# ERGO-Code/ipx

Hardware: AMD Instinct MI355X
Metric: kkt_solves_per_sec (higher is better)
Workload: dtype f64; 1 GPU; C3 synthetic LP m=1000000 n=2000000 8 nnz/col (nnz=16000000), KKTSolverDiag::Solve = diag-precond CR to tol=0.3*sqrt(mu), scaling spread s=1; rows of AI partitioned over 1 GPU(s); errflag=0

## Files before the change

ipx_amd/csrc/api.hip:

```cpp

#include <algorithm>
#include <map>
#include <thread>

#include "context.hpp"

namespace ipxk {

static thread_local std::string g_last_error;
void set_last_error(const std::string& msg) { g_last_error = msg; }

Context::~Context() {
    if (split) destroy_split(split);
    if (split_spare) destroy_split(split_spare);
    if (prepare_host) destroy_prepare_host(prepare_host);
    if (lu) destroy_lu(lu);
    if (maxvol) destroy_maxvol(maxvol);
    if (nmat) destroy_nmatrix(nmat);
    comm_destroy(this);
    if (h_state) (void)hipHostFree(h_state);
    if (h_cycle_done) (void)hipHostFree(h_cycle_done);
    if (ev_a) (void)hipEventDestroy(ev_a);
    if (ev_b) (void)hipEventDestroy(ev_b);
    for (hipEvent_t e : ev_window) (void)hipEventDestroy(e);
// ... 1200 lines not shown
        for (int i = 0; i < 48; i++) info[i] = 0;
        const SpmvLayout L = M.layout;
        info[0] = M.tile_base() != SpmvLayout::phased; info[2] = L == SpmvLayout::sortedfused; info[3] = M.nlong;
        info[4] = M.sliced.built; info[5] = M.sliced.R; info[6] = M.sliced.nslices; info[7] = M.sliced.nrb;
        info[8] = M.sliced.nrows_pad; info[9] = M.sliced.max_tile;
        { double d = M.sliced.dominant_fraction; memcpy(&info[10], &d, sizeof d); }
        info[11] = M.sorted.built; info[14] = M.sorted.nrb;
        info[15] = M.sorted.RB; info[16] = M.sorted.nrows_pad; info[17] = M.sorted.max_sub;
        info[20] = M.nnz;
        info[21] = M.P; info[22] = M.G; info[23] = (ipxint)M.RT * 1000000 + (ipxint)M.Q * 1000 + 0;
        info[24] = L == SpmvLayout::acc; info[25] = M.acc.built; info[26] = M.acc.nslices; info[27] = M.acc.nrb; info[28] = M.acc.RB;
        info[29] = M.acc.nrows_pad; info[30] = M.acc.slice_elems; info[31] = M.acc.nbatches; info[32] = M.acc.deferred;
        info[33] = L == SpmvLayout::accfused; info[34] = M.accf.built; info[35] = M.accf.nrb; info[36] = M.accf.RB; info[37] = M.accf.nbatches;
        info[38] = L == SpmvLayout::plain; info[39] = M.acc.nsteps;
        info[40] = M.acc.wide_units;
        if (create_ms) for (int i = 0; i < 4; i++) create_ms[i] = c->create_ms[i];
    });
}
int ipxk_layout_array(ipxk_context* c, int which, int array, void* out, ipxint cap, ipxint* nbytes) {
    return guarded([&] {
        IPXK_REQUIRE(c && nbytes && (which == 0 || which == 1), "bad argument");
        bind_device(c);
        const GatherMatrix& M = which == 0 ? c->Acols : c->Arows;
        const void* src = nullptr;
        size_t bytes = 0;
        const size_t ntiles = (size_t)M.sliced.nrb * M.sliced.nslices, nsorted = (size_t)M.sorted.nrb;
        const size_t nz = (size_t)M.nnz;
        switch (array) {
            case 0: src = M.sliced.tile_ptr.get(); bytes = M.sliced.built ? (ntiles + 1) * 4 : 0; break;
            case 1: src = M.sliced.cnt.get(); bytes = M.sliced.built ? ntiles * M.sliced.R : 0; break;
// ... 88 lines not shown
```

ipx_amd/csrc/context.hpp:

```cpp
#pragma once

#include "internal.hpp"
#include "device_utils.hpp"

struct ncclComm;

namespace ipxk {

constexpr int kPartialStride = kMaxPartials + 8;

enum PartialSlot {
    kPartRes0 = 0,
    kPartRes1,
    kPartPdot,
    kPartCdot,
    kPartRsdot,
    kPartScratch,
    kNumPartialSlots
};

struct Reordered {
    bool active = false;
    int levels = 0;
    int components = 0;
// ... 57 lines not shown
    DevBuf<int> schur_colptr;
    DevBuf<int> chol_info;
    DevBuf<unsigned char> dense_mask;
    std::vector<int> dense_rank_k;
    DevBuf<double> dense_W, dense_Wsend, dense_Wrecv;
    DevBuf<int> dense_Widx;

    DevBuf<double> v_rhs, v_lhs, v_residual, v_sresidual, v_step, v_Cstep, v_Cres, v_pCstep;
    DevBuf<double> v_resscale_in;
    DevBuf<double> partials;
    DevBuf<CrState> state;
    CrState* h_state = nullptr;
    DevBuf<double> hist;
    hipEvent_t ev_a = nullptr, ev_b = nullptr;
    std::vector<hipEvent_t> ev_window;

    DevBuf<double> resscale;
    DevBuf<double> k_a, k_b, k_x, k_y;
    DevBuf<double> k_tmp;
    bool kkt_diag_factorized = false;

    DevBuf<double> nw_rhs1, nw_rhs2;
    DevBuf<double> nw_in[10], nw_out[6];
    DevBuf<unsigned char> nw_state;

    DevBuf<double> it_x, it_xl, it_xu, it_y, it_zl, it_zu, it_partials;
    DevBuf<double> it_row, it_bnd, it_table;
    DevBuf<unsigned char> it_state;
    bool it_set = false;
    DevBuf<double> ipm[12];
// ... 67 lines not shown
void reorder_permute_weights(Context* c, const double* W_old, double* W_new);

void dense_lu_inverse(Context* c, int kb, const double* D, const double* invL, const double* invU, double* X, double* Xt, int refine = 0);

enum TimeKind { kTimeOp = 0, kTimePrecond = 1, kTimeB = 2, kTimeBt = 3, kNumTimeKinds = 4 };
void time_mark(Context* c, int kind, bool begin);
void time_start(Context* c, ipxk_times* times);
void time_collect(Context* c, ipxk_times* times);

const double* stage_in(Context* c, const double* p, size_t len, DevBuf<double>& buf);
double* stage_out(Context* c, double* p, size_t len, DevBuf<double>& buf);
void finish_out(Context* c, double* user, const double* dev, size_t len);

void normal_apply_dev(Context* c, const double* W, const double* rhs, double* lhs, int* ndot,
                      const int* done);
float time_normal_pair(Context* c, GatherMatrix& Ac, GatherMatrix& Ar);
void debug_single_pass(Context* c, int which, const double* x, double* out);

void prepare_dense_columns(Context* c);
void reset_dense_columns(Context* c);
void diag_factorize_dev(Context* c, const double* W, bool precond_dense_cols, ipxint* errflag);
int diag_apply_dev(Context* c, const double* rhs, double* lhs, int slot, const int* done);

struct CrResult { ipxint iter; ipxint errflag; };
CrResult pcr_solve_dev(Context* c, const double* rhs, double tol, const double* resscale,
                       ipxint maxiter, double* lhs, bool lhs_is_zero, ipxk_interrupt_fn interrupt,
                       void* user, double* hist_host, ipxint hist_cap, ipxk_times* times);
CrResult cr_solve_dev(Context* c, const double* rhs, double tol, const double* resscale,
                      ipxint maxiter, double* lhs, bool lhs_is_zero, ipxk_interrupt_fn interrupt,
                      void* user, double* hist_host, ipxint hist_cap, ipxk_times* times);
// ... 180 lines not shown
```

ipx_amd/csrc/cr.hip:

```cpp
#include <cmath>

#include "context.hpp"
#include "spmv_kernels.hpp"

namespace ipxk {

constexpr int kWindow = 2;

enum CrMode { kModePcrDiag = 0, kModePcrSmw = 1, kModePlain = 2 };

constexpr int kCrUnroll = 4;

struct CrVecs {
    int m;
    double* lhs;
    double* residual;
    double* sresidual;
    double* step;
    double* Cstep;
    double* Cres;
    double* pCstep;
    const double* resscale;
    const double* diag;
};
// ... 23 lines not shown
        st->maxiter = maxiter;
        st->k_started = 0;
        st->k_finished = 0;
        st->cdot[0] = st->cdot[1] = 0.0;
        st->rps[0] = r;
        st->rps[1] = 0.0;
        st->resnorm = 0.0;
        st->iter = 0;
        st->errflag = 0;
        st->done = 0;
        st->hist_cap = hist_cap;
        st->diag_rps_old = st->diag_rps_new = 0.0;
        st->mode = mode;
        st->alpha_pending = 0.0;
        st->k_pending = -1;
    }
}

struct CtlGroup {
    double q[kCrUnroll], r[kCrUnroll], sr[kCrUnroll], d[kCrUnroll], sc[kCrUnroll], s[kCrUnroll], l[kCrUnroll];
};
template <int MODE>
__device__ __forceinline__ void ctl_load(const CrVecs& v, int lazy, long long i0, long long stride, long long last, CtlGroup& g) {
#pragma unroll
    for (int u = 0; u < kCrUnroll; u++) {
        const long long i = min(i0 + u * stride, last);
        g.q[u] = v.Cstep[i];
        g.r[u] = v.residual[i];
        if (MODE != kModePlain) g.sr[u] = v.sresidual[i];
        if (MODE == kModePcrDiag) g.d[u] = v.diag[i];
// ... 208 lines not shown
    for (; i0 < v.m; i0 += kCrUnroll * stride) {
        DirGroup g{};
        dir_load<MODE, INIT>(v, src, owed, i0, stride, last, g);
        dir_update<MODE, INIT>(v, owed, alpha, beta, i0, stride, last, g, acc);
    }
    if (MODE != kModePcrSmw) {
        acc = block_reduce<SumOp>(acc, red);
        if (threadIdx.x == 0) pdot_partial[blockIdx.x] = acc;
    }
    if (blockIdx.x == 0 && threadIdx.x == 0) {
        st->cdot[(k + 1) & 1] = cdotnew;
        st->k_finished = k + 1;
    }
}

__global__ __launch_bounds__(kBlock) void cr_flush_update_kernel(const CrState* st, CrVecs v) {
    if (st->k_pending < 0 || st->k_pending != st->k_finished) return;
    const double alpha = st->alpha_pending;
    for (int i = blockIdx.x * kBlock + threadIdx.x; i < v.m; i += gridDim.x * kBlock) v.lhs[i] += alpha * v.step[i];
}

__global__ __launch_bounds__(kBlock) void finalize_scalar_kernel(PartRef ref, int op, double* out) {
    __shared__ double red[kBlock / 64 + 1];
    const double v = op == 1 ? reduce_partials<MaxOp>(ref, red)
                   : op == 2 ? reduce_partials<MinOp>(ref, red) : reduce_partials<SumOp>(ref, red);
    if (threadIdx.x == 0) *out = v;
}

__global__ void snapshot_done_kernel(const CrState* st, int* host_slot) {
    __hip_atomic_store(host_slot, st->done, __ATOMIC_RELAXED, __HIP_MEMORY_SCOPE_SYSTEM);
// ... 10 lines not shown
constexpr int kDoneRing = kWindow + 2;
constexpr int kDoneNow = 2 * kDoneRing;

static bool cr_lazy() {
    static const bool setting = [] { const char* e = getenv("IPXK_CR_LAZY"); return !e || atoi(e) != 0; }();
    return setting;
}

static bool cr_early() {
    static const bool setting = [] { const char* e = getenv("IPXK_CR_EARLY"); return !e || atoi(e) != 0; }();
    return setting;
}

static int cr_grid_cap() {
    static const int setting = [] { const char* e = getenv("IPXK_CR_GRID"); return e ? atoi(e) : 0; }();
    return setting;
}

static void ensure_comm_buffers(Context* c) {
    if (c->comm_scalars.size() < 64) c->comm_scalars.resize(64);
    if (c->comm_send.size() < (size_t)kNumPartialSlots) {
        c->comm_send.resize(kNumPartialSlots);
        IPXK_HIP(hipMemsetAsync(c->comm_send.get(), 0, sizeof(double) * kNumPartialSlots, c->stream));
    }
    const size_t need = (size_t)c->nranks * kNumPartialSlots;
    if (c->comm_gather.size() < need) c->comm_gather.resize(need);
}

struct Pub {
    Context* c;
// ... 69 lines not shown

struct CrOps {
    int mode;
    int (*applyC)(Context*, const double* rhs, double* lhs, const int* done);
};

static int applyC_normal(Context* c, const double* rhs, double* lhs, const int* done) {
    int np = 0;
    time_mark(c, kTimeOp, true);
    normal_apply_dev(c, c->W, rhs, lhs, &np, done);
    time_mark(c, kTimeOp, false);
    return np;
}
static int applyC_split(Context* c, const double* rhs, double* lhs, const int* done) {
    return split_apply_dev(c, rhs, lhs, done);
}

template <int MODE>
static CrResult run_cr(Context* c, const CrOps& ops, const double* rhs, double tol,
                       const double* resscale, ipxint maxiter, double* lhs, bool lhs_is_zero,
                       ipxk_interrupt_fn interrupt, void* user, double* hist_host, ipxint hist_cap,
                       ipxk_times* times) {
    ensure_workspaces(c);
    time_start(c, times);
    hipStream_t s = c->stream;
    const int m = (int)c->m;
    if (maxiter < 0) maxiter = (comm_active(c) ? c->m_global : c->m) + 100;
    if (hist_cap < 0) hist_cap = 0;
    if (!hist_host) hist_cap = 0;
    if (c->hist.size() < (size_t)hist_cap + 1) c->hist.resize((size_t)hist_cap + 1);
    CrState* st = c->state.get();
    int* done = &st->done;
    const int g = cr_grid_cap() > 0 ? std::min(vec_grid(m), cr_grid_cap()) : vec_grid(m);
    const Pub pub(c);
    for (int i = 0; i <= kDoneNow; i++) c->h_cycle_done[i] = 0;
    const bool multi = comm_active(c);
    const int lazy = cr_lazy() ? 1 : 0;
    const bool early = cr_early() && m > 0;
    const auto control = early ? cr_control_update_kernel<MODE, true> : cr_control_update_kernel<MODE, false>;
    const auto direction0 = early ? cr_direction_kernel<MODE, true, true> : cr_direction_kernel<MODE, true, false>;
    const auto direction = early ? cr_direction_kernel<MODE, false, true> : cr_direction_kernel<MODE, false, false>;
    int* done_now = multi ? nullptr : c->d_cycle_done + kDoneNow;
    if (multi) ensure_comm_buffers(c);

    CrVecs v;
    v.m = m; v.lhs = lhs; v.residual = c->v_residual.get(); v.sresidual = c->v_sresidual.get();
    v.step = c->v_step.get(); v.Cstep = c->v_Cstep.get(); v.Cres = c->v_Cres.get();
    v.pCstep = c->v_pCstep.get(); v.resscale = resscale; v.diag = c->reord.in_use ? c->reord.diagonal.get() : c->diagonal.get();

    IPXK_HIP(hipEventRecord(c->ev_a, s));

    if (lhs_is_zero) {
        hipLaunchKernelGGL(residual_init_kernel, dim3(g), dim3(kBlock), 0, s, m, rhs,
                           (const double*)nullptr, resscale, v.residual, c->part(kPartRes0));
    } else {
        ops.applyC(c, lhs, v.Cres, nullptr);
        hipLaunchKernelGGL(residual_init_kernel, dim3(g), dim3(kBlock), 0, s, m, rhs,
                           (const double*)v.Cres, resscale, v.residual, c->part(kPartRes0));
// ... 6 lines not shown
    const PartRef rsdot = MODE != kModePlain ? pub.ref(kPartRsdot, nrsdot) : PartRef{nullptr, 0, 1};
    hipLaunchKernelGGL(cr_init_state_kernel, dim3(1), dim3(kBlock), 0, s, st, tol, (long long)maxiter,
                       (long long)hist_cap, rsdot, (int)MODE);
    const double* csrc = MODE == kModePlain ? v.residual : v.sresidual;
    int ncdot = ops.applyC(c, csrc, v.Cres, nullptr);
    pub.publish(kPartCdot, ncdot, 0);
    hipLaunchKernelGGL(direction0, dim3(g), dim3(kBlock), 0, s, st, v,
                       pub.ref(kPartCdot, ncdot), c->part(kPartPdot));
    int npdot = g;
    if (MODE == kModePcrSmw) npdot = diag_apply_dev(c, v.Cstep, v.pCstep, kPartPdot, nullptr);
    pub.publish(kPartPdot, npdot, 0);
    const PartRef pdot_ref = pub.ref(kPartPdot, npdot);

    ipxint interrupt_flag = 0, my_interrupt = 0;
    bool agreed_done = false, tail = false;
    for (long long cycle = 0;; cycle++) {
        const long long k0 = cycle * 5;
        if (k0 > maxiter) break;
        if (cycle >= kWindow) {
            const long long cw = cycle - kWindow;
            IPXK_HIP(hipEventSynchronize(c->ev_window[cw % (kWindow + 1)]));
            if (*(volatile int*)(c->h_cycle_done + cw % kDoneRing)) { agreed_done = true; break; }
            if (multi) {
                const int agreed = *(volatile int*)(c->h_cycle_done + kDoneRing + cw % kDoneRing);
                if (agreed != 0) { interrupt_flag = agreed; break; }
            }
        }
        if (interrupt && cycle > 0) {
            my_interrupt = interrupt(user);
            if (!multi && my_interrupt != 0) { interrupt_flag = my_interrupt; break; }
        }
        for (long long k = k0; k < k0 + 5 && k <= maxiter; k++) {
            if (done_now && *(volatile int*)(c->h_cycle_done + kDoneNow)) tail = true;
            if (tail) break;
            hipLaunchKernelGGL(control, dim3(g), dim3(kBlock), 0, s, st, v,
                               res0, res1, pdot_ref, rsdot, c->part(kPartRes0), c->part(kPartRes1),
                               c->hist.get(), lazy, done_now);
            ncdot = ops.applyC(c, csrc, v.Cres, done);
            pub.publish(kPartCdot, ncdot, 0, ((k + 1) & 1) ? kPartRes1 : kPartRes0, g, 1);
            hipLaunchKernelGGL(direction, dim3(g), dim3(kBlock), 0, s, st, v,
                               pub.ref(kPartCdot, ncdot), c->part(kPartPdot));
            if (MODE == kModePcrSmw) diag_apply_dev(c, v.Cstep, v.pCstep, kPartPdot, done);
            if (MODE != kModePlain && (k + 1) % 5 == 0) {
                diag_apply_dev(c, v.residual, v.sresidual, kPartRsdot, done);
                pub.publish(kPartPdot, npdot, 0, kPartRsdot, nrsdot, 0);
            } else {
                pub.publish(kPartPdot, npdot, 0);
            }
        }
        if (multi) {
            double* flags = c->comm_scalars.get() + 56;
            hipLaunchKernelGGL(cycle_flags_kernel, dim3(1), dim3(1), 0, s, st, (double)my_interrupt, flags);
            comm_allreduce_max(c, flags, 2);
            hipLaunchKernelGGL(snapshot_flags_kernel, dim3(1), dim3(1), 0, s, flags, c->d_cycle_done + cycle % kDoneRing,
                               c->d_cycle_done + kDoneRing + cycle % kDoneRing);
        } else {
            hipLaunchKernelGGL(snapshot_done_kernel, dim3(1), dim3(1), 0, s, st, c->d_cycle_done + cycle % kDoneRing);
        }
        IPXK_HIP(hipEventRecord(c->ev_window[cycle % (kWindow + 1)], s));
    }
    if (lazy) hipLaunchKernelGGL(cr_flush_update_kernel, dim3(g), dim3(kBlock), 0, s, st, v);
    IPXK_HIP(hipEventRecord(c->ev_b, s));
    IPXK_HIP(hipMemcpyAsync(c->h_state, st, sizeof(CrState), hipMemcpyDeviceToHost, s));
    IPXK_HIP(hipStreamSynchronize(s));
    IPXK_HIP(hipGetLastError());
    comm_check(c);

    if (multi && agreed_done && !c->h_state->done)
        throw Error(IPXK_E_HIP, "ranks of a partitioned solve diverged (another rank finished the CR loop, this one did not)");
    CrResult res;
    if (c->h_state->done) {
        res.iter = c->h_state->iter;
        res.errflag = c->h_state->errflag;
    } else {
        res.iter = c->h_state->k_finished;
        res.errflag = interrupt_flag;
    }
    if (hist_cap > 0) {
        long long nh = c->h_state->done && c->h_state->errflag != 204 ? res.iter + 1 : res.iter;
        if (!c->h_state->done) nh = c->h_state->k_started;
        if (nh > hist_cap) nh = hist_cap;
// ... 71 lines not shown
```

ipx_amd/csrc/device_utils.hpp:

```cpp
#pragma once

#include <hip/hip_runtime.h>

#include <climits>

#include "internal.hpp"

#define IPXK_GRID_STRIDE(i, n) for (int64_t i = (int64_t)blockIdx.x * blockDim.x + threadIdx.x; i < (n); i += (int64_t)gridDim.x * blockDim.x)

namespace ipxk {

template <class T>
__global__ void fill_kernel(int64_t n, T v, T* __restrict__ a) { IPXK_GRID_STRIDE(i, n) a[i] = v; }

template <int kThreads>
__global__ __launch_bounds__(kThreads) void scan_u32_kernel(int n, const unsigned* __restrict__ in, unsigned* __restrict__ out) {
    __shared__ unsigned wsum[kThreads / 64];
    __shared__ unsigned carry;
    const int tid = threadIdx.x, lane = tid & 63, wave = tid >> 6;
    if (tid == 0) carry = 0;
    __syncthreads();
    for (int base = 0; base < n; base += kThreads) {
        const int i = base + tid;
        const unsigned v = i < n ? in[i] : 0u;
// ... 118 lines not shown
__device__ __forceinline__ void block_argmax(double& v, int& i) {
    __shared__ double sv[kThreads / 64];
    __shared__ int si[kThreads / 64];
    wave_argmax(v, i);
    if ((threadIdx.x & 63) == 0) { sv[threadIdx.x >> 6] = v; si[threadIdx.x >> 6] = i; }
    __syncthreads();
    if (threadIdx.x == 0)
        for (int k = 1; k < kThreads / 64; k++) take_larger(v, i, sv[k], si[k]);
}
template <int kBest>
__device__ __forceinline__ Partial<kBest> load_partial(int nparts, const Partial<kBest>* part) {
    return (int)threadIdx.x < nparts ? part[threadIdx.x] : partial_identity<kBest>();
}

template <class Op>
__device__ __forceinline__ double block_reduce(double v, double* scratch) {
    const int lane = threadIdx.x & 63, wave = threadIdx.x >> 6;
    v = wave_reduce<Op>(v);
    __syncthreads();
    if (lane == 0) scratch[wave] = v;
    __syncthreads();
    double r = scratch[0];
#pragma unroll
    for (int w = 1; w < kBlock / 64; w++) r = Op::apply(r, scratch[w]);
    return r;
}

struct PartRef {
    const double* p;
    int count;
    int stride;
};

constexpr int kPartialsPerThread = kMaxPartials / kBlock;

__device__ __forceinline__ void load_partials(PartRef part, double (&v)[kPartialsPerThread]) {
    const int last = max(part.count - 1, 0);
#pragma unroll
    for (int j = 0; j < kPartialsPerThread; j++)
        v[j] = part.p[(size_t)min((int)threadIdx.x + j * kBlock, last) * part.stride];
}
template <class Op>
__device__ __forceinline__ double fold_partials(PartRef part, const double (&v)[kPartialsPerThread]) {
    double r = Op::identity();
#pragma unroll
    for (int j = 0; j < kPartialsPerThread; j++)
        if ((int)threadIdx.x + j * kBlock < part.count) r = Op::apply(r, v[j]);
    for (int i = threadIdx.x + kMaxPartials; i < part.count; i += kBlock)
        r = Op::apply(r, part.p[(size_t)i * part.stride]);
    return r;
}

template <class Op>
__device__ __forceinline__ double reduce_partials(PartRef part, double* scratch) {
    double v[kPartialsPerThread];
    load_partials(part, v);
    return block_reduce<Op>(fold_partials<Op>(part, v), scratch);
}

template <class OpA, class OpB>
__device__ __forceinline__ void block_reduce2(double& va, double& vb, double* scratch_a, double* scratch_b) {
    const int lane = threadIdx.x & 63, wave = threadIdx.x >> 6;
    va = wave_reduce<OpA>(va);
    vb = wave_reduce<OpB>(vb);
    __syncthreads();
    if (lane == 0) { scratch_a[wave] = va; scratch_b[wave] = vb; }
    __syncthreads();
    double ra = scratch_a[0], rb = scratch_b[0];
#pragma unroll
    for (int w = 1; w < kBlock / 64; w++) { ra = OpA::apply(ra, scratch_a[w]); rb = OpB::apply(rb, scratch_b[w]); }
    va = ra;
    vb = rb;
}
template <class OpA, class OpB>
__device__ __forceinline__ void reduce_partials2(PartRef a, PartRef b, double* scratch_a, double* scratch_b, double& ra,
                                                 double& rb) {
    double va[kPartialsPerThread], vb[kPartialsPerThread];
    load_partials(a, va);
    load_partials(b, vb);
    ra = fold_partials<OpA>(a, va);
    rb = fold_partials<OpB>(b, vb);
    block_reduce2<OpA, OpB>(ra, rb, scratch_a, scratch_b);
}

}
```

ipx_amd/csrc/internal.hpp:

```cpp
#pragma once

#include <hip/hip_runtime.h>

#include <chrono>
#include <cstdint>
#include <cstdio>
#include <cstdlib>
#include <algorithm>
#include <cstring>
#include <functional>
#include <memory>
#include <stdexcept>
#include <string>
#include <type_traits>
#include <vector>

#include "../../include/ipx_kkt_hip.h"

namespace ipxk {

struct Error : std::runtime_error {
    int code;
    Error(int c, const std::string& what) : std::runtime_error(what), code(c) {}
};
// ... 281 lines not shown
    double tol;
    long long maxiter;
    long long k_started;
    long long k_finished;
    double cdot[2];
    double rps[2];
    double resnorm;
    long long iter;
    int errflag;
    int done;
    long long hist_cap;
    double diag_rps_old, diag_rps_new;
    int mode;
    double alpha_pending;
    long long k_pending;
};

struct MvScalars {
    int jn;
    double weight;
    int pmax, jb;
    double vmax, weight_recomp, colscale_jn, invscale_pmax, pivot_col;
    int used_pmax, eta_nnz;
    double pivot_row;
    int eta_total;
};

template <int kBest>
struct Partial { double v[kBest]; int i[kBest]; double s; int c; };
using MvPart = Partial<1>;
// ... 90 lines not shown
```

ipx_amd/csrc/spmv.hip:

```cpp
#include <algorithm>
#include <cstdio>
#include <cstdlib>
#include <string>
#include <utility>

#include "context.hpp"
#include "spmv_kernels.hpp"

namespace ipxk {

int slice_elems() {
    static int cached = 0;
    if (!cached) {
        int kb = 1024;
        if (const char* e = getenv("IPXK_SLICE_KB")) kb = atoi(e) > 0 ? atoi(e) : kb;
        cached = kb * 128;
    }
    return cached;
}

int64_t phase_slice(int64_t ncols_) {
    constexpr int kMaxPhases = 64;
    int64_t slice = slice_elems();
    if ((ncols_ + slice - 1) / slice > kMaxPhases) slice = (ncols_ + kMaxPhases - 1) / kMaxPhases;
// ... 297 lines not shown
        const int np = launch_spmv(R.Arows, R.tcols.get(), e2, ndot ? c->part(kPartCdot) : nullptr, done, c->stream);
        if (ndot) *ndot = np;
        return;
    }
    double* stage = comm_rows(c) ? comm_stage(c, (size_t)n) : nullptr;
    EpiScale e1{{}, W, stage ? stage : c->tcols.get()};
    launch_spmv(c->Acols, rhs, e1, nullptr, done, c->stream);
    if (stage) comm_allreduce_sum_staged(c, c->tcols.get(), (size_t)n);
    else if (comm_rows(c)) comm_allreduce_sum(c, c->tcols.get(), (size_t)n);
    EpiNormalRows e2{{}, W + n, rhs, lhs};
    const int np = launch_spmv(c->Arows, c->tcols.get(), e2, ndot ? c->part(kPartCdot) : nullptr,
                               done, c->stream);
    if (ndot) *ndot = np;
}

void debug_single_pass(Context* c, int which, const double* x, double* out) {
    if (which == 1) {
        EpiScale e1{{}, c->W, out};
        launch_spmv(c->Acols, x, e1, nullptr, nullptr, c->stream);
    } else {
        EpiNormalRows e2{{}, c->W + c->n, out, out};
        launch_spmv(c->Arows, x, e2, nullptr, nullptr, c->stream);
    }
}

}
```

ipx_amd/csrc/spmv_kernels.hpp:

```cpp
#pragma once

#include <type_traits>

#include "device_utils.hpp"
#include "internal.hpp"

namespace ipxk {

constexpr int kLdsDoubles = kChunkNnz + kChunkNnz / 32;

__device__ __forceinline__ int lds_slot(int q) { return q + (q >> 5); }

template <class Epi, class = void>
struct EpiRow {
    struct In {};
    static __device__ __forceinline__ In load(const Epi&, long long) { return In{}; }
    static __device__ __forceinline__ double init(const Epi& e, long long r, const In&) { return e.init((int)r); }
    static __device__ __forceinline__ void finish(const Epi& e, long long r, const In&, double acc, double& dot) { e.finish((int)r, acc, dot); }
};
template <class Epi>
struct EpiRow<Epi, std::void_t<typename Epi::In>> {
    using In = typename Epi::In;
    static __device__ __forceinline__ In load(const Epi& e, long long r) { return e.load(r); }
    static __device__ __forceinline__ double init(const Epi& e, long long, const In& in) { return e.init(in); }
// ... 911 lines not shown
    }
    const size_t lds = (size_t)W.RB * sizeof(double);
    const int ntiles = W.nrb * W.nslices, G = acc_persist_grid(W.nslices);
    const dim3 pgrid(std::min(G, ntiles));
    if (G > 0 && W.wide)
        hipLaunchKernelGGL((spmv_acc_persist_kernel<Prod, true>), pgrid, dim3(kAccThreads), lds, s, W, W.tile_step, W.steps, W.wide_start,
                           reinterpret_cast<const acc_u32x4*>(W.wide), x, done);
    else if (G > 0)
        hipLaunchKernelGGL((spmv_acc_persist_kernel<Prod, false>), pgrid, dim3(kAccThreads), lds, s, W, W.tile_step, W.steps,
                           (const unsigned*)nullptr, (const acc_u32x4*)nullptr, x, done);
    else hipLaunchKernelGGL((spmv_acc_tile_kernel<Prod>), dim3(ntiles), dim3(kAccThreads), lds, s, W, x, done);
}

template <class Epi, bool MASKED = false, bool COMPACT = false>
inline void launch_spmv_sliced(const GatherMatrix& M, const double* x, const Epi& epi, double* dot_partials,
                               const int* done, hipStream_t s) {
    static_assert(!(MASKED && COMPACT), "the compacted copy needs no mask");
    const SlicedView V = M.sliced_view(COMPACT ? 2 : MASKED ? 1 : 0);
    const size_t lds = (size_t)(M.sliced.max_tile + M.sliced.max_tile / 32 + 1) * sizeof(double);
    const dim3 grid(V.nrb * V.nslices), block(kBlock);
    if (V.nslices == 1) {
        const dim3 fgrid(M.fused_grid());
        if (V.R == kBlock * 4) hipLaunchKernelGGL((spmv_sliced_tile_kernel<Epi, 4, true, MASKED>), fgrid, block, lds, s, V, x, epi, dot_partials, done);
        else if (V.R == kBlock * 2) hipLaunchKernelGGL((spmv_sliced_tile_kernel<Epi, 2, true, MASKED>), fgrid, block, lds, s, V, x, epi, dot_partials, done);
        else hipLaunchKernelGGL((spmv_sliced_tile_kernel<Epi, 1, true, MASKED>), fgrid, block, lds, s, V, x, epi, dot_partials, done);
    } else {
        if (V.R == kBlock * 4) hipLaunchKernelGGL((spmv_sliced_tile_kernel<Epi, 4, false, MASKED>), grid, block, lds, s, V, x, epi, dot_partials, done);
        else if (V.R == kBlock * 2) hipLaunchKernelGGL((spmv_sliced_tile_kernel<Epi, 2, false, MASKED>), grid, block, lds, s, V, x, epi, dot_partials, done);
        else hipLaunchKernelGGL((spmv_sliced_tile_kernel<Epi, 1, false, MASKED>), grid, block, lds, s, V, x, epi, dot_partials, done);
        launch_combine(V, epi, dot_partials, done, s);
    }
}

template <class Epi, bool MASKED = false>
inline int launch_spmv(const GatherMatrix& M, const double* x, const Epi& epi, double* dot_partials,
                       const int* done, hipStream_t s) {
    switch (MASKED ? M.tile_base() : M.layout) {
        case SpmvLayout::accfused: {
            const AccView W = M.acc_fused_view();
            static bool lds_attr_set = false;
            if (!lds_attr_set) {
                IPXK_HIP(hipFuncSetAttribute(reinterpret_cast<const void*>(spmv_acc_fused_kernel<Epi>), hipFuncAttributeMaxDynamicSharedMemorySize,
                                             (int)(kAccMaxRows * sizeof(double))));
                lds_attr_set = true;
            }
            hipLaunchKernelGGL((spmv_acc_fused_kernel<Epi>), dim3(W.nrb), dim3(kAccThreads), (size_t)W.RB * sizeof(double), s, W, x, epi, dot_partials, done);
// ... 56 lines not shown
```

ipx_amd/kkt.py:

```python
import ctypes as C
import os
import subprocess

import numpy as np

HERE = os.path.dirname(os.path.abspath(__file__))
LIB_PATH = os.path.join(HERE, "lib", "libipx_kkt_hip.so")

i64, f64 = np.int64, np.float64
c_i64, c_f64 = C.c_int64, C.c_double
P_i64, P_f64 = C.POINTER(C.c_int64), C.POINTER(C.c_double)
INTERRUPT_FN = C.CFUNCTYPE(c_i64, C.c_void_p)

POINTER_HOST, POINTER_DEVICE = 0, 1
NONBASIC_FIXED, NONBASIC, BASIC, BASIC_FREE = -2, -1, 0, 1

EXPORTS = [
    "ipxk_last_error", "ipxk_device_count", "ipxk_create", "ipxk_destroy", "ipxk_set_pointer_mode",
    "ipxk_set_stream", "ipxk_synchronize", "ipxk_set_profiling", "ipxk_set_interrupt", "ipxk_reset_solver_state", "ipxk_get_reorder_info", "ipxk_get_reordering", "ipxk_num_dense_cols", "ipxk_get_rowwise",
    "ipxk_normal_prepare", "ipxk_normal_apply", "ipxk_diag_factorize", "ipxk_diag_apply",
    "ipxk_diag_get", "ipxk_pcr_solve", "ipxk_cr_diagnostics", "ipxk_kkt_diag_factorize", "ipxk_kkt_diag_solve",
    "ipxk_kkt_diag_get", "ipxk_split_prepare", "ipxk_split_rescale", "ipxk_split_apply", "ipxk_forward_solve",
    "ipxk_backward_solve", "ipxk_solve_dense", "ipxk_split_levels", "ipxk_cr_solve",
    "ipxk_kkt_basis_solve", "ipxk_newton_solve", "ipxk_iterate_set", "ipxk_iterate_get", "ipxk_iterate_update",
# ... 282 lines not shown
        a, b, w = C.c_int64(0), C.c_int64(0), C.c_double(0.0)
        self._check(self.lib.ipxk_split_inverse_stats(self.h, C.byref(a), C.byref(b), C.byref(w)))
        return a.value, b.value, w.value

    def split_inverse_refined(self):
        return int(self.lib.ipxk_split_inverse_refined(self.h))

    def layout_info(self, which):
        info = (C.c_int64 * 48)()
        ms = (C.c_double * 4)()
        self._check(self.lib.ipxk_layout_info(self.h, which, info, ms))
        keys = ("use_sliced", None, "use_sorted_fused", "nlong", "sliced_built", "R", "nslices", "nrb", "nrows_pad",
                "max_tile", "dominant_bits", "sorted_built", None, None, "so_nrb", "so_RB", "so_nrows_pad",
                "so_max_sub", None, None, "nnz", "P", "G", "RTQ", "use_acc", "acc_built", "acc_nslices", "acc_nrb",
                "acc_RB", "acc_nrows_pad", "acc_slice_elems", "acc_nbatches", "acc_deferred", "use_acc_fused", "accf_built", "accf_nrb", "accf_RB",
                "accf_nbatches", "use_plain", "acc_nsteps", "acc_wide_units")
        d = {k: int(v) for k, v in zip(keys, info) if k is not None}
        d["dominant_fraction"] = float(np.array([d.pop("dominant_bits")], dtype=np.int64).view(np.float64)[0])
        return d, [float(v) for v in ms]

    def layout_array(self, which, array):
        dt = (np.uint32, np.uint8, np.int32, np.float64, np.uint32, np.uint8, np.uint32, np.float64, np.int32, np.int32, np.float64,
              np.uint32, np.uint32, np.uint32, np.float64, np.uint32, np.uint32, np.uint32, np.float64, np.int32, np.int32,
              np.uint32, np.uint32, np.uint32, np.uint32)[array]
        nb = C.c_int64(0)
        self._check(self.lib.ipxk_layout_array(self.h, which, array, None, 0, C.byref(nb)))
        out = np.zeros(nb.value // np.dtype(dt).itemsize, dtype=dt)
        if nb.value:
            self._check(self.lib.ipxk_layout_array(self.h, which, array, out.ctypes.data_as(C.c_void_p), nb.value, C.byref(nb)))
            self._check(self.lib.ipxk_synchronize(self.h))
        return out
# ... 472 lines not shown
```

Before: 63.55 solves/s.

## Fuse SpMV combine, CR direction and control into one grid-barrier tail kernel

Adds a persistent-style cr_tail_kernel for the diagonal-preconditioned CR loop. It folds the sliced SpMV partial sums (the combine step), the cdot reduction, the direction update and the next iteration's control and residual update into a single launch. Cross-workgroup reductions use a hierarchical atomic grid barrier, and the launch is guarded by an occupancy check so that all workgroups are resident. The aim is to remove several kernel launches and round trips through global memory per iteration. The cost is the risk of barrier deadlock, which is handled by a spin limit and an error path, plus added complexity. It is on by default and can be disabled with IPXK_CR_TAIL=0.

Result: faster. 66.16 solves/s (median of 4 runs) (+4.1%).

```diff
diff --git a/ipx_amd/csrc/api.hip b/ipx_amd/csrc/api.hip
--- a/ipx_amd/csrc/api.hip
+++ b/ipx_amd/csrc/api.hip
@@ -1238,6 +1238,7 @@
         info[33] = L == SpmvLayout::accfused; info[34] = M.accf.built; info[35] = M.accf.nrb; info[36] = M.accf.RB; info[37] = M.accf.nbatches;
         info[38] = L == SpmvLayout::plain; info[39] = M.acc.nsteps;
         info[40] = M.acc.wide_units;
+        info[41] = c->tail_launches;
         if (create_ms) for (int i = 0; i < 4; i++) create_ms[i] = c->create_ms[i];
     });
 }
diff --git a/ipx_amd/csrc/context.hpp b/ipx_amd/csrc/context.hpp
--- a/ipx_amd/csrc/context.hpp
+++ b/ipx_amd/csrc/context.hpp
@@ -95,6 +95,10 @@
     DevBuf<double> hist;
     hipEvent_t ev_a = nullptr, ev_b = nullptr;
     std::vector<hipEvent_t> ev_window;
+    DevBuf<unsigned> tail_bar;
+    int tail_resident[4] = {0, 0, 0, 0};
+    int tail_nwg = 0;
+    long long tail_launches = 0;
 
     DevBuf<double> resscale;
     DevBuf<double> k_a, k_b, k_x, k_y;
@@ -192,6 +196,10 @@
 
 void normal_apply_dev(Context* c, const double* W, const double* rhs, double* lhs, int* ndot,
                       const int* done);
+struct EpiNormalRows;
+bool normal_apply_stops(const Context* c);
+void normal_apply_tiles_dev(Context* c, const double* W, const double* rhs, double* lhs, const int* done, SlicedView* V,
+                            EpiNormalRows* epi);
 float time_normal_pair(Context* c, GatherMatrix& Ac, GatherMatrix& Ar);
 void debug_single_pass(Context* c, int which, const double* x, double* out);
 
diff --git a/ipx_amd/csrc/cr.hip b/ipx_amd/csrc/cr.hip
--- a/ipx_amd/csrc/cr.hip
+++ b/ipx_amd/csrc/cr.hip
@@ -61,6 +61,7 @@
         st->mode = mode;
         st->alpha_pending = 0.0;
         st->k_pending = -1;
+        st->tail_error = 0;
     }
 }
 
@@ -299,6 +300,224 @@
     }
 }
 
+constexpr int kTailRows = 4;
+constexpr int kTailVBlocks = 4;
+constexpr int kTailThreads = kTailVBlocks * kBlock;
+constexpr int kTailSpinLimit = 1 << 22;
+constexpr int kTailBarWords = 10 * 32;
+constexpr int kTailParts = kMaxWorkgroups / kBlock;
+
+struct TailBar {
+    unsigned* words;
+    unsigned nwg, ngroups;
+};
+
+__device__ __forceinline__ void tail_arrive(const TailBar& B, unsigned target) {
+    __syncthreads();
+    if (threadIdx.x == 0) {
+        const unsigned grp = blockIdx.x % B.ngroups, n = B.nwg / B.ngroups + (grp < B.nwg % B.ngroups ? 1u : 0u);
+        if (__hip_atomic_fetch_add(B.words + grp * 32, 1u, __ATOMIC_RELAXED, __HIP_MEMORY_SCOPE_AGENT) + 1u == target * n &&
+            __hip_atomic_fetch_add(B.words + 8 * 32, 1u, __ATOMIC_RELAXED, __HIP_MEMORY_SCOPE_AGENT) + 1u == target * B.ngroups)
+            __hip_atomic_store(B.words + 9 * 32, target, __ATOMIC_RELAXED, __HIP_MEMORY_SCOPE_AGENT);
+    }
+}
+__device__ __forceinline__ bool tail_wait(const TailBar& B, unsigned target, CrState* st, int* host_done, int* ok_lds) {
+    if (threadIdx.x == 0) {
+        int ok = 1, spins = 0;
+        while ((int)(__hip_atomic_load(B.words + 9 * 32, __ATOMIC_RELAXED, __HIP_MEMORY_SCOPE_AGENT) - target) < 0) {
+            __builtin_amdgcn_s_sleep(1);
+            if (++spins > kTailSpinLimit ||
+                ((spins & 255) == 0 && __hip_atomic_load(&st->tail_error, __ATOMIC_RELAXED, __HIP_MEMORY_SCOPE_AGENT))) {
+                __hip_atomic_store(&st->tail_error, 1, __ATOMIC_RELAXED, __HIP_MEMORY_SCOPE_AGENT);
+                __hip_atomic_store(&st->done, 1, __ATOMIC_RELAXED, __HIP_MEMORY_SCOPE_AGENT);
+                if (host_done) __hip_atomic_store(host_done, 1, __ATOMIC_RELAXED, __HIP_MEMORY_SCOPE_SYSTEM);
+                ok = 0;
+                break;
+            }
+        }
+        *ok_lds = ok;
+    }
+    __syncthreads();
+    return *ok_lds != 0;
+}
+
+template <int NS>
+__global__ __launch_bounds__(kTailThreads) void cr_tail_kernel(
+    CrState* st, CrVecs v, const double* partial, int nrows_pad, int nslices, const double* wI, TailBar bar, int G,
+    double* cdot_part, double* pdot_part, PartRef res0, PartRef res1, double* res_next0, double* res_next1, double* hist,
+    int* host_done, int with_control) {
+    __shared__ double red[kTailVBlocks][kBlock / 64 + 1], red2[kTailVBlocks][kBlock / 64 + 1];
+    __shared__ int bar_ok;
+    const int vbl = threadIdx.x / kBlock, vt = threadIdx.x % kBlock;
+    const int vb = blockIdx.x * kTailVBlocks + vbl;
+    const bool vlive = vb < G, writer = vb == 0 && vt == 0;
+    const long long stride = (long long)G * kBlock, last = v.m - 1;
+    const long long first = (long long)min(vb, G - 1) * kBlock + vt;
+
+    __shared__ unsigned top[2];
+    const int done = st->done, tail_error = __hip_atomic_load(&st->tail_error, __ATOMIC_RELAXED, __HIP_MEMORY_SCOPE_AGENT);
+    const unsigned gen_read = __hip_atomic_load(bar.words + 9 * 32, __ATOMIC_RELAXED, __HIP_MEMORY_SCOPE_AGENT);
+    const long long k_started = st->k_started, k_pending = st->k_pending, maxiter = st->maxiter, hist_cap = st->hist_cap;
+    const double cdot0 = st->cdot[0], cdot1 = st->cdot[1], alpha_owed = st->alpha_pending, tol = st->tol;
+
+    constexpr int B = NS ? NS : 8, R = B == 8 ? 2 : 4;
+    const int ns = NS ? NS : nslices;
+    long long rc[kTailRows];
+    bool live[kTailRows];
+    double y[kTailRows], cres[kTailRows];
+#pragma unroll
+    for (int j = 0; j < kTailRows; j++) {
+        live[j] = vlive && first + j * stride <= last;
+        rc[j] = min(first + j * stride, last);
+    }
+    double dot = 0.0;
+#pragma unroll
+    for (int j0 = 0; j0 < kTailRows; j0 += R) {
+        double w[R], t[R][B];
+#pragma unroll
+        for (int j = 0; j < R; j++) {
+            y[j0 + j] = v.sresidual[rc[j0 + j]];
+            w[j] = wI ? wI[rc[j0 + j]] : 0.0;
+        }
+#pragma unroll
+        for (int j = 0; j < R; j++)
+#pragma unroll
+            for (int u = 0; u < B; u++) t[j][u] = __builtin_nontemporal_load(partial + (size_t)min(u, ns - 1) * nrows_pad + rc[j0 + j]);
+        asm volatile("" ::: "memory");
+        __builtin_amdgcn_sched_barrier(0);
+        double acc[R];
+#pragma unroll
+        for (int j = 0; j < R; j++) acc[j] = live[j0 + j] ? (wI ? y[j0 + j] * w[j] : 0.0) : 0.0;
+        for (int s0 = 0; s0 < ns; s0 += B) {
+            if (s0 > 0) {
+#pragma unroll
+                for (int j = 0; j < R; j++)
+#pragma unroll
+                    for (int u = 0; u < B; u++)
+                        t[j][u] = __builtin_nontemporal_load(partial + (size_t)min(s0 + u, ns - 1) * nrows_pad + rc[j0 + j]);
+            }
+#pragma unroll
+            for (int j = 0; j < R; j++)
+#pragma unroll
+                for (int u = 0; u < B; u++)
+                    if (NS || s0 + u < ns) acc[j] = acc[j] + t[j][u];
+        }
+#pragma unroll
+        for (int j = 0; j < R; j++) {
+            cres[j0 + j] = acc[j];
+            if (live[j0 + j]) dot += y[j0 + j] * acc[j];
+        }
+    }
+    if (threadIdx.x == 0) {
+        top[0] = (done != 0 || tail_error != 0) ? 1u : 0u;
+        top[1] = gen_read;
+    }
+    __syncthreads();
+    if (top[0]) return;
+    const unsigned gen0 = top[1];
+    dot = block_reduce_at<SumOp>(dot, red[vbl], vt);
+    if (vt == 0 && vlive) __hip_atomic_store(cdot_part + vb, dot, __ATOMIC_RELAXED, __HIP_MEMORY_SCOPE_AGENT);
+    asm volatile("s_waitcnt vmcnt(0)" ::: "memory");
+
+    double s[kTailRows], cs[kTailRows], l[kTailRows], d[kTailRows];
+    tail_arrive(bar, gen0 + 1u);
+#pragma unroll
+    for (int j = 0; j < kTailRows; j++) {
+        s[j] = v.step[rc[j]];
+        cs[j] = v.Cstep[rc[j]];
+        l[j] = v.lhs[rc[j]];
+        d[j] = v.diag[rc[j]];
+    }
+    if (!tail_wait(bar, gen0 + 1u, st, host_done, &bar_ok)) return;
+
+    const PartRef cdot_ref{cdot_part, G, 1};
+    double pc[kTailParts];
+    load_partials_at<true>(cdot_ref, pc, vt);
+    const double cdotnew = block_reduce_at<SumOp>(fold_partials_at<SumOp, true>(cdot_ref, pc, vt), red[vbl], vt);
+    const long long k = k_started - 1;
+    const double beta = cdotnew / ((k & 1) ? cdot1 : cdot0);
+    const bool owed = k_pending == k;
+    double q[kTailRows];
+    double acc = 0.0;
+#pragma unroll
+    for (int j = 0; j < kTailRows; j++) {
+        q[j] = cs[j];
+        if (!live[j]) continue;
+        const long long i = rc[j];
+        if (owed) v.lhs[i] = l[j] + alpha_owed * s[j];
+        const double p = y[j] + beta * s[j];
+        q[j] = cres[j] + beta * cs[j];
+        v.step[i] = p;
+        v.Cstep[i] = q[j];
+        acc += (q[j] / d[j]) * q[j];
+    }
+    acc = block_reduce_at<SumOp>(acc, red[vbl], vt);
+    if (vt == 0 && vlive) __hip_atomic_store(pdot_part + vb, acc, __ATOMIC_RELAXED, __HIP_MEMORY_SCOPE_AGENT);
+    if (writer) {
+        st->cdot[(k + 1) & 1] = cdotnew;
+        st->k_finished = k + 1;
+    }
+    if (!with_control) return;
+    asm volatile("s_waitcnt vmcnt(0)" ::: "memory");
+
+    const long long k1 = k + 1;
+    const PartRef res_ref = (k1 & 1) ? res1 : res0;
+    double r[kTailRows], sc[kTailRows], pr[kTailParts];
+    tail_arrive(bar, gen0 + 2u);
+#pragma unroll
+    for (int j = 0; j < kTailRows; j++) {
+        r[j] = v.residual[rc[j]];
+        sc[j] = v.resscale ? v.resscale[rc[j]] : 0.0;
+    }
+    load_partials_at(res_ref, pr, vt);
+    if (!tail_wait(bar, gen0 + 2u, st, host_done, &bar_ok)) return;
+
+    const PartRef pdot_ref{pdot_part, G, 1};
+    double pp[kTailParts];
+    load_partials_at<true>(pdot_ref, pp, vt);
+    double resnorm = fold_partials_at<MaxOp>(res_ref, pr, vt), pdot = fold_partials_at<SumOp, true>(pdot_ref, pp, vt);
+    block_reduce2_at<MaxOp, SumOp>(resnorm, pdot, red[vbl], red2[vbl], vt);
+    if (writer && k1 < hist_cap) hist[k1] = resnorm;
+    int errflag = -1;
+    double alpha = 0.0;
+    if (resnorm <= tol) errflag = 0;
+    else if (k1 == maxiter) errflag = 201;
+    else if (cdotnew <= 0.0) errflag = 202;
+    else if (pdot <= 0.0) errflag = 203;
+    else {
+        alpha = cdotnew / pdot;
+        if (!isfinite(alpha)) errflag = 205;
+    }
+    if (errflag >= 0) {
+        if (writer) {
+            st->errflag = errflag;
+            st->iter = k1;
+            st->resnorm = resnorm;
+            st->done = 1;
+            if (host_done) __hip_atomic_store(host_done, 1, __ATOMIC_RELAXED, __HIP_MEMORY_SCOPE_SYSTEM);
+        }
+        return;
+    }
+    double mx = 0.0;
+#pragma unroll
+    for (int j = 0; j < kTailRows; j++) {
+        if (!live[j]) continue;
+        const long long i = rc[j];
+        const double rn = r[j] - alpha * q[j];
+        v.residual[i] = rn;
+        v.sresidual[i] = y[j] - alpha * (q[j] / d[j]);
+        mx = MaxOp::apply(mx, fabs(v.resscale ? sc[j] * rn : rn));
+    }
+    mx = block_reduce_at<MaxOp>(mx, red[vbl], vt);
+    if (vt == 0 && vlive) ((k1 & 1) ? res_next0 : res_next1)[vb] = mx;
+    if (writer) {
+        st->k_started = k1 + 1;
+        st->resnorm = resnorm;
+        st->alpha_pending = alpha;
+        st->k_pending = k1;
+    }
+}
+
 __global__ __launch_bounds__(kBlock) void cr_flush_update_kernel(const CrState* st, CrVecs v) {
     if (st->k_pending < 0 || st->k_pending != st->k_finished) return;
     const double alpha = st->alpha_pending;
@@ -339,6 +558,11 @@
 
 static int cr_grid_cap() {
     static const int setting = [] { const char* e = getenv("IPXK_CR_GRID"); return e ? atoi(e) : 0; }();
+    return setting;
+}
+
+static bool cr_tail() {
+    static const bool setting = [] { const char* e = getenv("IPXK_CR_TAIL"); return !e || atoi(e) != 0; }();
     return setting;
 }
 
@@ -438,6 +662,54 @@
 }
 static int applyC_split(Context* c, const double* rhs, double* lhs, const int* done) {
     return split_apply_dev(c, rhs, lhs, done);
+}
+
+static int tail_instance(int ns) { return combine_generic() ? 3 : ns == 2 ? 0 : ns == 4 ? 1 : ns == 8 ? 2 : 3; }
+static const void* tail_function(int inst) {
+    switch (inst) {
+        case 0: return reinterpret_cast<const void*>(cr_tail_kernel<2>);
+        case 1: return reinterpret_cast<const void*>(cr_tail_kernel<4>);
+        case 2: return reinterpret_cast<const void*>(cr_tail_kernel<8>);
+        default: return reinterpret_cast<const void*>(cr_tail_kernel<0>);
+    }
+}
+
+static bool tail_plan(Context* c, int m, int g, bool multi, int lazy, bool early, TailBar* bar) {
+    if (!cr_tail() || multi || !lazy || !early || !combine_early() || !normal_apply_stops(c)) return false;
+    if (combine_grid_for(m) != g || ((int64_t)m + (int64_t)g * kBlock - 1) / ((int64_t)g * kBlock) > kTailRows) return false;
+    const GatherMatrix& Ar = c->reord.in_use ? c->reord.Arows : c->Arows;
+    const int inst = tail_instance(Ar.sliced_view(0).nslices), nwg = (g + kTailVBlocks - 1) / kTailVBlocks;
+    if (c->tail_resident[inst] == 0) {
+        int per_cu = 0, cus = 0;
+        IPXK_HIP(hipOccupancyMaxActiveBlocksPerMultiprocessor(&per_cu, tail_function(inst), kTailThreads, 0));
+        IPXK_HIP(hipDeviceGetAttribute(&cus, hipDeviceAttributeMultiprocessorCount, c->device));
+        c->tail_resident[inst] = per_cu * cus > 0 ? per_cu * cus : -1;
+    }
+    if (c->tail_resident[inst] < nwg) return false;
+    if (c->tail_bar.size() == 0 || c->tail_nwg != nwg) {
+        if (c->tail_bar.size() == 0) c->tail_bar.resize(kTailBarWords);
+        IPXK_HIP(hipMemsetAsync(c->tail_bar.get(), 0, kTailBarWords * sizeof(unsigned), c->stream));
+        c->tail_nwg = nwg;
+    }
+    *bar = TailBar{c->tail_bar.get(), (unsigned)nwg, (unsigned)std::min(nwg, 8)};
+    return true;
+}
+
+static void launch_tail(Context* c, CrState* st, const CrVecs& v, const SlicedView& V, const EpiNormalRows& e, const TailBar& bar,
+                        int g, const PartRef& res0, const PartRef& res1, int* host_done, int with_control) {
+    const dim3 grid(bar.nwg), block(kTailThreads);
+    const auto go = [&](auto kernel) {
+        hipLaunchKernelGGL(kernel, grid, block, 0, c->stream, st, v, (const double*)V.partial, V.nrows_pad, V.nslices, e.wI, bar, g,
+                           c->part(kPartCdot), c->part(kPartPdot), res0, res1, c->part(kPartRes0), c->part(kPartRes1),
+                           c->hist.get(), host_done, with_control);
+    };
+    switch (tail_instance(V.nslices)) {
+        case 0: go(cr_tail_kernel<2>); break;
+        case 1: go(cr_tail_kernel<4>); break;
+        case 2: go(cr_tail_kernel<8>); break;
+        default: go(cr_tail_kernel<0>); break;
+    }
+    c->tail_launches++;
 }
 
 template <int MODE>
@@ -466,6 +738,10 @@
     const auto direction = early ? cr_direction_kernel<MODE, false, true> : cr_direction_kernel<MODE, false, false>;
     int* done_now = multi ? nullptr : c->d_cycle_done + kDoneNow;
     if (multi) ensure_comm_buffers(c);
+    TailBar bar{};
+    bool fused = false;
+    if constexpr (MODE == kModePcrDiag) fused = m > 0 && tail_plan(c, m, g, multi, lazy, early, &bar);
+    c->tail_launches = 0;
 
     CrVecs v;
     v.m = m; v.lhs = lhs; v.residual = c->v_residual.get(); v.sresidual = c->v_sresidual.get();
@@ -502,6 +778,7 @@
 
     ipxint interrupt_flag = 0, my_interrupt = 0;
     bool agreed_done = false, tail = false;
+    bool ctl_in_tail = false;
     for (long long cycle = 0;; cycle++) {
         const long long k0 = cycle * 5;
         if (k0 > maxiter) break;
@@ -521,9 +798,24 @@
         for (long long k = k0; k < k0 + 5 && k <= maxiter; k++) {
             if (done_now && *(volatile int*)(c->h_cycle_done + kDoneNow)) tail = true;
             if (tail) break;
-            hipLaunchKernelGGL(control, dim3(g), dim3(kBlock), 0, s, st, v,
-                               res0, res1, pdot_ref, rsdot, c->part(kPartRes0), c->part(kPartRes1),
-                               c->hist.get(), lazy, done_now);
+            if (!ctl_in_tail)
+                hipLaunchKernelGGL(control, dim3(g), dim3(kBlock), 0, s, st, v,
+                                   res0, res1, pdot_ref, rsdot, c->part(kPartRes0), c->part(kPartRes1),
+                                   c->hist.get(), lazy, done_now);
+            if constexpr (MODE == kModePcrDiag) {
+                if (fused) {
+                    const bool refresh = (k + 1) % 5 == 0;
+                    SlicedView V;
+                    EpiNormalRows e2;
+                    time_mark(c, kTimeOp, true);
+                    normal_apply_tiles_dev(c, c->W, csrc, v.Cres, done, &V, &e2);
+                    time_mark(c, kTimeOp, false);
+                    ctl_in_tail = !refresh && k != maxiter;
+                    launch_tail(c, st, v, V, e2, bar, g, res0, res1, done_now, ctl_in_tail ? 1 : 0);
+                    if (refresh) diag_apply_dev(c, v.residual, v.sresidual, kPartRsdot, done);
+                    continue;
+                }
+            }
             ncdot = ops.applyC(c, csrc, v.Cres, done);
             pub.publish(kPartCdot, ncdot, 0, ((k + 1) & 1) ? kPartRes1 : kPartRes0, g, 1);
             hipLaunchKernelGGL(direction, dim3(g), dim3(kBlock), 0, s, st, v,
@@ -553,6 +845,11 @@
     IPXK_HIP(hipStreamSynchronize(s));
     IPXK_HIP(hipGetLastError());
     comm_check(c);
+    if (c->h_state->tail_error) {
+        IPXK_HIP(hipMemsetAsync(c->tail_bar.get(), 0, kTailBarWords * sizeof(unsigned), s));
+        IPXK_HIP(hipStreamSynchronize(s));
+        throw Error(IPXK_E_HIP, "the fused tail of the CR loop timed out at a grid barrier (IPXK_CR_TAIL=0 runs the loop without it)");
+    }
 
     if (multi && agreed_done && !c->h_state->done)
         throw Error(IPXK_E_HIP, "ranks of a partitioned solve diverged (another rank finished the CR loop, this one did not)");
diff --git a/ipx_amd/csrc/device_utils.hpp b/ipx_amd/csrc/device_utils.hpp
--- a/ipx_amd/csrc/device_utils.hpp
+++ b/ipx_amd/csrc/device_utils.hpp
@@ -156,8 +156,8 @@
 }
 
 template <class Op>
-__device__ __forceinline__ double block_reduce(double v, double* scratch) {
-    const int lane = threadIdx.x & 63, wave = threadIdx.x >> 6;
+__device__ __forceinline__ double block_reduce_at(double v, double* scratch, int tid) {
+    const int lane = tid & 63, wave = tid >> 6;
     v = wave_reduce<Op>(v);
     __syncthreads();
     if (lane == 0) scratch[wave] = v;
@@ -167,6 +167,8 @@
     for (int w = 1; w < kBlock / 64; w++) r = Op::apply(r, scratch[w]);
     return r;
 }
+template <class Op>
+__device__ __forceinline__ double block_reduce(double v, double* scratch) { return block_reduce_at<Op>(v, scratch, threadIdx.x); }
 
 struct PartRef {
     const double* p;
@@ -176,21 +178,31 @@
 
 constexpr int kPartialsPerThread = kMaxPartials / kBlock;
 
-__device__ __forceinline__ void load_partials(PartRef part, double (&v)[kPartialsPerThread]) {
+template <bool AGENT = false, int N = kPartialsPerThread>
+__device__ __forceinline__ void load_partials_at(PartRef part, double (&v)[N], int tid) {
     const int last = max(part.count - 1, 0);
 #pragma unroll
-    for (int j = 0; j < kPartialsPerThread; j++)
-        v[j] = part.p[(size_t)min((int)threadIdx.x + j * kBlock, last) * part.stride];
+    for (int j = 0; j < N; j++) {
+        const double* p = part.p + (size_t)min(tid + j * kBlock, last) * part.stride;
+        v[j] = AGENT ? __hip_atomic_load(p, __ATOMIC_RELAXED, __HIP_MEMORY_SCOPE_AGENT) : *p;
+    }
+}
+__device__ __forceinline__ void load_partials(PartRef part, double (&v)[kPartialsPerThread]) { load_partials_at(part, v, threadIdx.x); }
+template <class Op, bool AGENT = false, int N = kPartialsPerThread>
+__device__ __forceinline__ double fold_partials_at(PartRef part, const double (&v)[N], int tid) {
+    double r = Op::identity();
+#pragma unroll
+    for (int j = 0; j < N; j++)
+        if (tid + j * kBlock < part.count) r = Op::apply(r, v[j]);
+    for (int i = tid + N * kBlock; i < part.count; i += kBlock) {
+        const double* p = part.p + (size_t)i * part.stride;
+        r = Op::apply(r, AGENT ? __hip_atomic_load(p, __ATOMIC_RELAXED, __HIP_MEMORY_SCOPE_AGENT) : *p);
+    }
+    return r;
 }
 template <class Op>
 __device__ __forceinline__ double fold_partials(PartRef part, const double (&v)[kPartialsPerThread]) {
-    double r = Op::identity();
-#pragma unroll
-    for (int j = 0; j < kPartialsPerThread; j++)
-        if ((int)threadIdx.x + j * kBlock < part.count) r = Op::apply(r, v[j]);
-    for (int i = threadIdx.x + kMaxPartials; i < part.count; i += kBlock)
-        r = Op::apply(r, part.p[(size_t)i * part.stride]);
-    return r;
+    return fold_partials_at<Op>(part, v, threadIdx.x);
 }
 
 template <class Op>
@@ -201,8 +213,8 @@
 }
 
 template <class OpA, class OpB>
-__device__ __forceinline__ void block_reduce2(double& va, double& vb, double* scratch_a, double* scratch_b) {
-    const int lane = threadIdx.x & 63, wave = threadIdx.x >> 6;
+__device__ __forceinline__ void block_reduce2_at(double& va, double& vb, double* scratch_a, double* scratch_b, int tid) {
+    const int lane = tid & 63, wave = tid >> 6;
     va = wave_reduce<OpA>(va);
     vb = wave_reduce<OpB>(vb);
     __syncthreads();
@@ -213,6 +225,10 @@
     for (int w = 1; w < kBlock / 64; w++) { ra = OpA::apply(ra, scratch_a[w]); rb = OpB::apply(rb, scratch_b[w]); }
     va = ra;
     vb = rb;
+}
+template <class OpA, class OpB>
+__device__ __forceinline__ void block_reduce2(double& va, double& vb, double* scratch_a, double* scratch_b) {
+    block_reduce2_at<OpA, OpB>(va, vb, scratch_a, scratch_b, threadIdx.x);
 }
 template <class OpA, class OpB>
 __device__ __forceinline__ void reduce_partials2(PartRef a, PartRef b, double* scratch_a, double* scratch_b, double& ra,
diff --git a/ipx_amd/csrc/internal.hpp b/ipx_amd/csrc/internal.hpp
--- a/ipx_amd/csrc/internal.hpp
+++ b/ipx_amd/csrc/internal.hpp
@@ -319,6 +319,7 @@
     int mode;
     double alpha_pending;
     long long k_pending;
+    int tail_error;
 };
 
 struct MvScalars {
diff --git a/ipx_amd/csrc/spmv.hip b/ipx_amd/csrc/spmv.hip
--- a/ipx_amd/csrc/spmv.hip
+++ b/ipx_amd/csrc/spmv.hip
@@ -335,6 +335,24 @@
     if (ndot) *ndot = np;
 }
 
+bool normal_apply_stops(const Context* c) {
+    if (comm_active(c)) return false;
+    return spmv_ends_in_combine(c->reord.in_use ? c->reord.Arows : c->Arows);
+}
+
+void normal_apply_tiles_dev(Context* c, const double* W, const double* rhs, double* lhs, const int* done, SlicedView* V,
+                            EpiNormalRows* epi) {
+    const int64_t n = c->n;
+    const bool re = c->reord.in_use;
+    Reordered& R = c->reord;
+    const double* w = re ? R.W.get() : W;
+    double* t = re ? R.tcols.get() : c->tcols.get();
+    EpiScale e1{{}, w, t};
+    launch_spmv(re ? R.Acols : c->Acols, rhs, e1, nullptr, done, c->stream);
+    *epi = EpiNormalRows{{}, w + n, rhs, lhs};
+    *V = launch_spmv_tiles(re ? R.Arows : c->Arows, t, *epi, done, c->stream);
+}
+
 void debug_single_pass(Context* c, int which, const double* x, double* out) {
     if (which == 1) {
         EpiScale e1{{}, c->W, out};
diff --git a/ipx_amd/csrc/spmv_kernels.hpp b/ipx_amd/csrc/spmv_kernels.hpp
--- a/ipx_amd/csrc/spmv_kernels.hpp
+++ b/ipx_amd/csrc/spmv_kernels.hpp
@@ -949,7 +949,7 @@
 
 template <class Epi, bool MASKED = false, bool COMPACT = false>
 inline void launch_spmv_sliced(const GatherMatrix& M, const double* x, const Epi& epi, double* dot_partials,
-                               const int* done, hipStream_t s) {
+                               const int* done, hipStream_t s, SlicedView* stop = nullptr) {
     static_assert(!(MASKED && COMPACT), "the compacted copy needs no mask");
     const SlicedView V = M.sliced_view(COMPACT ? 2 : MASKED ? 1 : 0);
     const size_t lds = (size_t)(M.sliced.max_tile + M.sliced.max_tile / 32 + 1) * sizeof(double);
@@ -963,8 +963,26 @@
         if (V.R == kBlock * 4) hipLaunchKernelGGL((spmv_sliced_tile_kernel<Epi, 4, false, MASKED>), grid, block, lds, s, V, x, epi, dot_partials, done);
         else if (V.R == kBlock * 2) hipLaunchKernelGGL((spmv_sliced_tile_kernel<Epi, 2, false, MASKED>), grid, block, lds, s, V, x, epi, dot_partials, done);
         else hipLaunchKernelGGL((spmv_sliced_tile_kernel<Epi, 1, false, MASKED>), grid, block, lds, s, V, x, epi, dot_partials, done);
-        launch_combine(V, epi, dot_partials, done, s);
-    }
+        if (stop) *stop = V;
+        else launch_combine(V, epi, dot_partials, done, s);
+    }
+}
+
+inline bool spmv_ends_in_combine(const GatherMatrix& M) {
+    return M.nlong == 0 && (M.layout == SpmvLayout::acc || (M.layout == SpmvLayout::sliced && M.sliced.nslices > 1));
+}
+template <class Epi>
+inline SlicedView launch_spmv_tiles(const GatherMatrix& M, const double* x, const Epi& epi, const int* done, hipStream_t s) {
+    SlicedView C{};
+    if (M.layout == SpmvLayout::acc) {
+        const AccView W = M.acc_view();
+        launch_acc_tiles<Epi>(W, x, done, s);
+        C = M.sliced_view(0);
+        C.nrows_pad = W.nrows_pad; C.partial = W.partial;
+    } else {
+        launch_spmv_sliced<Epi>(M, x, epi, nullptr, done, s, &C);
+    }
+    return C;
 }
 
 template <class Epi, bool MASKED = false>
diff --git a/ipx_amd/kkt.py b/ipx_amd/kkt.py
--- a/ipx_amd/kkt.py
+++ b/ipx_amd/kkt.py
@@ -320,7 +320,7 @@
                 "max_tile", "dominant_bits", "sorted_built", None, None, "so_nrb", "so_RB", "so_nrows_pad",
                 "so_max_sub", None, None, "nnz", "P", "G", "RTQ", "use_acc", "acc_built", "acc_nslices", "acc_nrb",
                 "acc_RB", "acc_nrows_pad", "acc_slice_elems", "acc_nbatches", "acc_deferred", "use_acc_fused", "accf_built", "accf_nrb", "accf_RB",
-                "accf_nbatches", "use_plain", "acc_nsteps", "acc_wide_units")
+                "accf_nbatches", "use_plain", "acc_nsteps", "acc_wide_units", "cr_tail_launches")
         d = {k: int(v) for k, v in zip(keys, info) if k is not None}
         d["dominant_fraction"] = float(np.array([d.pop("dominant_bits")], dtype=np.int64).view(np.float64)[0])
         return d, [float(v) for v in ms]
```
